# karpathy/minbpe

Hardware: AMD Instinct MI355X
Metric: BPE merges/sec (higher is better)
Workload: dtype int32; 1 GPU; regex1g: RegexTokenizer.train, 1 GB synth seed 2, vocab 32000; mode=default, parallelism=single

## Files before the change

### minbpe_amd/csrc/api/api_basic.hip

```cpp

extern "C" {

const char *bpe_version(void) { return "minbpe_amd libbpe_hip 0.1 (gfx950)"; }

const char *bpe_last_error(bpe_ctx *ctx) { return ctx ? ctx->err.c_str() : g_create_err.c_str(); }

int bpe_create(int device_id, bpe_ctx **out) {
    if (!out) return fail(nullptr, BPE_E_ARG, "out is NULL");
    *out = nullptr;
    int ndev = 0;
    hipError_t e = hipGetDeviceCount(&ndev);
    if (e != hipSuccess || ndev == 0)
        return fail(nullptr, BPE_E_HIP, "no HIP device available: %s",
                    e != hipSuccess ? hipGetErrorString(e) : "device count is 0");
    if (device_id < 0 || device_id >= ndev)
        return fail(nullptr, BPE_E_ARG, "device %d out of range (%d devices)", device_id, ndev);
    bpe_ctx *c = new bpe_ctx();
    c->device = device_id;
    auto bail = [&](const char *what, hipError_t er) {
        int rc = fail(nullptr, BPE_E_HIP, "%s failed: %s", what, hipGetErrorString(er));
        delete c;
        return rc;
    };
    if ((e = hipSetDevice(device_id)) != hipSuccess) return bail("hipSetDevice", e);
    hipDeviceProp_t prop;
    if ((e = hipGetDeviceProperties(&prop, device_id)) != hipSuccess)
        return bail("hipGetDeviceProperties", e);
    c->num_cus = prop.multiProcessorCount > 0 ? prop.multiProcessorCount : 256;
    if (prop.sharedMemPerBlock < (size_t)LEAN_LDS_BYTES) c->lean = 0;
    if ((e = hipStreamCreateWithFlags(&c->stream, hipStreamNonBlocking)) != hipSuccess)
        return bail("hipStreamCreate", e);
    c->own_stream = true;
    for (const void *fn : {(const void *)k_pair_count_lds, (const void *)k_pair_count_bytes, (const void *)k_pair_count_h32})
        if ((e = hipFuncSetAttribute(fn, hipFuncAttributeMaxDynamicSharedMemorySize, PC_LDS_BYTES)) != hipSuccess)
            return bail("hipFuncSetAttribute(dynamic LDS)", e);
    if ((e = hipFuncSetAttribute((const void *)k_load_count, hipFuncAttributeMaxDynamicSharedMemorySize, LC_LDS_BYTES)) != hipSuccess)
        return bail("hipFuncSetAttribute(dynamic LDS)", e);
    if ((e = hipFuncSetAttribute((const void *)bpe::bpe_g4::k_index_build, hipFuncAttributeMaxDynamicSharedMemorySize,
                                 bpe::bpe_g4::IDX_H * 4)) != hipSuccess)
        return bail("hipFuncSetAttribute(dynamic LDS)", e);
    if ((e = hipMalloc((void **)&c->d_st, sizeof(DevState))) != hipSuccess) return bail("hipMalloc", e);
    if ((e = hipMalloc((void **)&c->d_scratch, 8 * sizeof(unsigned long long))) != hipSuccess)
        return bail("hipMalloc", e);
    *out = c;
    return BPE_OK;
}

void bpe_destroy(bpe_ctx *c) {
    if (!c) return;
    (void)hipSetDevice(c->device);
    if (c->stream) (void)hipStreamSynchronize(c->stream);
    if (c->comm) (void)bpe_comm_destroy(c);
    for (ProfEv &ev : c->prof_open) {
        (void)hipEventDestroy(ev.e0);
// ... 448 lines not shown
```

### minbpe_amd/csrc/api/api_train.hip

```cpp

extern "C" {

int bpe_train(bpe_ctx *c, int32_t num_merges, int32_t *pairs_out, uint64_t *counts_out,
              double *iter_ms_out, uint64_t *len_out, int32_t *n_done) {
    if (!c || num_merges < 0) return fail(c, BPE_E_ARG, "bad arguments");
    if (!c->have_bytes) return fail(c, BPE_E_STATE, "bpe_load_bytes first");
    if (c->dp_active) return fail(c, BPE_E_STATE, "bpe_dp_end first");
    static const bool timing = getenv("BPE_TIMING") != nullptr;
    auto now = [] { return std::chrono::steady_clock::now(); };
    auto t_begin = now();
    struct ProfIterReset {
        bpe_ctx *c;
        ~ProfIterReset() { c->prof_iter = -1; }
    } prof_iter_reset{c};
    if (n_done) *n_done = 0;
    HIPCHK(c, hipSetDevice(c->device));
    TRY(ensure_table(c, 256u + (uint32_t)num_merges));
    TRY(ensure_rec(c, std::max(num_merges, 1)));
    memset(c->h_rec, 0, sizeof(IterRec) * (size_t)std::max(num_merges, 1));
    TRY(ensure_srec(c));
    const bool delta = (c->mode == 1);
    EventList ev_list;
    std::vector<hipEvent_t> &evs = ev_list.v;
    struct EvSpan {
// ... 26 lines not shown
    const bool slots = delta && c->use_slots && c->merge_impl == 0;
    const bool form2 = slots && c->use_slots == 2;
    c->idx_live = false;
    c->idx_rebuild = false;
    c->last_count = ~0ull;
    c->n_sparse = c->n_dense = c->n_index_builds = 0;
    c->n_lean = c->n_deferred = 0;
    c->n_steps = c->n_full = c->n_chained = 0;
    c->n_fused = 0;
    static const char *stamp_path = getenv("BPE_STEP_STAMPS");
    const size_t stamp_bytes = (size_t)STEP_STAMP_RING * (3 * 16 + 256 * 2) * sizeof(unsigned long long);
    if (stamp_path) {
        if (!c->d_step_stamps) HIPCHK(c, hipMalloc((void **)&c->d_step_stamps, stamp_bytes));
        HIPCHK(c, hipMemsetAsync(c->d_step_stamps, 0, stamp_bytes, c->stream));
    }
    if (c->d_step_bar) {
        HIPCHK(c, hipMemsetAsync(c->d_step_bar, 0, 256, c->stream));
        c->step_bar_target = 0;
    }
    c->rows_pending = false;
    c->sum_valid = false;
    enum { U_GENERAL = 0, U_LEAN = 1, U_CHAIN = 2 };
    struct Unit {
        int kind;
        int iter;
        uint32_t step;
        uint8_t hdr_flip;
        uint8_t aa_indexed;
        uint8_t pass_kind;
        int ev;
// ... 303 lines not shown
            HIPCHK(c, hipEventElapsedTime(&ms, evs[(size_t)prev], evs[(size_t)sp.ev]));
            for (int j = 0; j < sp.k; j++)
                if (sp.first + j < done) iter_ms_out[sp.first + j] = ms / sp.k;
            prev = sp.ev;
        }
    }
    TRY(prof_drain(c));
    if (stamp_path && c->d_step_stamps) {
        std::vector<unsigned long long> h(stamp_bytes / sizeof(unsigned long long));
        HIPCHK(c, hipMemcpy(h.data(), c->d_step_stamps, stamp_bytes, hipMemcpyDeviceToHost));
        if (FILE *f = fopen(stamp_path, "wb")) {
            fwrite(h.data(), 1, stamp_bytes, f);
            fclose(f);
        }
    }
    if (timing) {
        auto ms = [](auto a, auto b) { return std::chrono::duration<double, std::milli>(b - a).count(); };
        fprintf(stderr, "[bpe_train] %d merges: setup+enqueue of the first pass %.2f ms, loop %.2f ms, drain %.2f ms, "
                        "re-pack + timers %.2f ms\n", done, ms(t_begin, t_loop), ms(t_loop, t_drain), ms(t_drain, t_tail),
                ms(t_tail, now()));
    }
    if (n_done) *n_done = done;
    return rc;
}

}
```

### minbpe_amd/csrc/bpe_device.h

```cpp
#pragma once
#include <stdint.h>

namespace bpe {

constexpr uint32_t FLAG = 0x80000000u;
constexpr uint32_t IDMASK = 0x03FFFFFFu;
constexpr int WSHIFT = 26;
constexpr uint32_t WMASK = 0x7C000000u;
constexpr uint32_t NWMASK = ~WMASK;
constexpr uint32_t INVALID_WORD = 0xFFFFFFFFu;
constexpr uint32_t EMPTY_KEY = 0xFFFFFFFFu;
constexpr unsigned long long NOPOS = ~0ull;

constexpr int MT = 256;
#define BPE_GEOMETRY(NS, MJV, IDXH_LOG2)                                                                         \
    namespace NS {                                                                                               \
    constexpr int MJ = MJV;                            \
    constexpr int WAVE_SPAN = MJ * 256;                                                                          \
    constexpr int TILE = (MT / 64) * WAVE_SPAN;  \
                      \
    constexpr int TILE2 = WAVE_SPAN;                                                                             \
                                  \
    constexpr uint32_t IDX_H = 1u << IDXH_LOG2;                                                                  \
    constexpr int IDX_SHIFT = 32 - IDXH_LOG2;                                                                    \
    }
BPE_GEOMETRY(bpe_g4, 4, 15)
#ifndef BPE_G1_IDXH_LOG2
#define BPE_G1_IDXH_LOG2 13
#endif
BPE_GEOMETRY(bpe_g1, 1, BPE_G1_IDXH_LOG2)
constexpr int TILE2_MAX = 1024, TILE2_MIN = 256;

constexpr int PC_BITS = 14;
constexpr int PC_THREADS = 1024;
constexpr int PC_LDS_BYTES = 131072;
constexpr int PCB_ROUND = 61440;

constexpr int TIE_CAP = 96;
constexpr int ARGMAX_ROWS = 2048;
constexpr uint32_t TIE_WINDOW0 = 0;
constexpr int TIE_BLOCKS = 256;
constexpr int ROW_BLOCKS = 64;
constexpr int DELTA_REPL = 256;
constexpr int DELTA_SKEW = 64;
constexpr int REMOVED_STRIDE = 64;
constexpr int LDSD_CAP = 1920;
// ... 201 lines not shown
```

### minbpe_amd/csrc/kernels/k_chain.hip

```cpp
#include <hip/hip_runtime.h>
#include <stdint.h>

#include "../bpe_device.h"

namespace bpe {
namespace BPE_G {

constexpr uint32_t CH_EX_CAP = 2048;

__device__ __forceinline__ int chain_match(const uint32_t *pa, const uint32_t *pb, uint32_t K, uint32_t w0, uint32_t w1) {
    const uint32_t x = w0 & IDMASK, y = w1 & NWMASK;
    int hit = -1;
    for (uint32_t p = 0; p < K; p++)
        if (x == pa[p] && y == pb[p]) hit = (int)p;
    return (w0 == INVALID_WORD) ? -1 : hit;
}

constexpr uint32_t CH_DCAP = 1024;
constexpr uint32_t CH_SD = 2 * CH_DCAP + 2;
__device__ __forceinline__ void chain_slot_load(const AbArgs &A, const uint32_t t, uint4 (&rv)[MJ], uint4 &hv) {
    const int lane = lane_id();
    const uint32_t *src = A.b0 + (size_t)t * TILE2;
#pragma unroll
    for (int j = 0; j < MJ; j++) rv[j] = *reinterpret_cast<const uint4 *>(src + j * 256 + lane * 4);
    hv = (lane & 1) ? make_uint4(INVALID_WORD, INVALID_WORD, 0u, 0u) : make_uint4(INVALID_WORD, INVALID_WORD, INVALID_WORD, 0u);
    const long long hi = 2ll * (long long)t - 2 + lane;
    if (lane < 6 && hi >= 0 && hi < 2ll * (long long)A.T) hv = reinterpret_cast<const uint4 *>(A.hdr_in)[hi];
}
template <bool DENSE, bool THROUGH = false>
__device__ __forceinline__ void merge_chain_wave(uint32_t *__restrict__ out, uint32_t *__restrict__ sd, const uint32_t t, const AbArgs &A,
                                                 const uint32_t *pa, const uint32_t *pb, const uint32_t *pb1,
                                                 const uint32_t K, const uint32_t z0, const uint32_t brep,
                                                 uint4 (&rv)[MJ], const uint4 hv,
                                                 const uint32_t *ph = nullptr, const uint32_t hm = 0,
                                                 const uint32_t tl_in = 0xFFFFFFFFu) {
    const int lane = lane_id();
    const uint32_t Tl = tl_in != 0xFFFFFFFFu ? tl_in : min(A.T, A.st->tlive);
    const uint32_t *src;
    const uint32_t meta = bcast(hv.w, 2);
    const uint32_t len = meta & 0x7FFFFFFFu, buf = meta >> 31;
    auto keep_header = [&]() {
        if (DENSE && (lane == 2 || lane == 3)) reinterpret_cast<uint4 *>(A.hdr_out)[2 * (size_t)t + (lane - 2)] = hv;
    };
    if (len == 0) {
        keep_header();
        return;
    }
    if (buf) {
        src = A.b1 + (size_t)t * TILE2;
#pragma unroll
        for (int j = 0; j < MJ; j++) rv[j] = *reinterpret_cast<const uint4 *>(src + j * 256 + lane * 4);
    }
    const uint32_t first = bcast(hv.x, 2);
    uint32_t halo0 = bcast(hv.x, 4), halo1 = bcast(hv.y, 4), halo2 = bcast(hv.z, 4);
    uint32_t prev2 = bcast(hv.x, 1), prev1 = bcast(hv.y, 1);
    uint32_t tprev = t - 1;
    uint32_t tnext = t + 1;
    {
        const uint32_t nlen = bcast(hv.w, 4) & 0x7FFFFFFFu, plen = bcast(hv.w, 0) & 0x7FFFFFFFu;
        if ((t + 1 < Tl && nlen < 3) || (t > 0 && plen < 2)) {
            uint32_t ctx[7] = {0, 0, 0, 0, 0, 0, 0};
            if (lane == 0) slot_context_walk(A.hdr_in, t, Tl, ctx);
            halo0 = bcast(ctx[0], 0);
            halo1 = bcast(ctx[1], 0);
            halo2 = bcast(ctx[2], 0);
            prev2 = bcast(ctx[3], 0);
            prev1 = bcast(ctx[4], 0);
            tprev = bcast(ctx[5], 0);
            tnext = bcast(ctx[6], 0);
        }
    }
    auto at = [&](int q, uint32_t own) -> uint32_t {
        const int d = q - (int)len;
        return d < 0 ? own : (d == 0 ? halo0 : (d == 1 ? halo1 : (d == 2 ? halo2 : INVALID_WORD)));
    };
// ... 11 lines not shown
            x[j][1] = at(q0 + 1, rv[j].y);
            x[j][2] = at(q0 + 2, rv[j].z);
            x[j][3] = at(q0 + 3, rv[j].w);
        }
    }
    uint32_t tail[3];
#pragma unroll
    for (int i = 0; i < 3; i++) tail[i] = at(TILE2 + i, 0u);
    uint32_t rb[MJ], jc[MJ], valid[MJ];
#pragma unroll
    for (int j = 0; j < MJ; j++) {
        rb[j] = 0;
        jc[j] = 0;
    }
    uint32_t s = 0;
    uint32_t ia[MJ];
#pragma unroll
    for (int j = 0; j < MJ; j++) ia[j] = 0;
    uint32_t ip = 0;
    if (hm) {
        auto code = [&](uint32_t w) -> uint32_t {
            const uint32_t id = w & IDMASK;
            const uint32_t e = ph[(__umul24(id, hm) >> 8) & 255u];
            return (e >> 8) == id ? (e & 15u) : 0u;
        };
#pragma unroll
        for (int j = 0; j < MJ; j++) {
#pragma unroll
            for (int k = 0; k < 4; k++) ia[j] |= code(x[j][k]) << (4 * k);
        }
        ip = code(prev1);
    } else {
        for (uint32_t p = 0; p < K; p++) {
            const uint32_t a = pa[p];
#pragma unroll
            for (int j = 0; j < MJ; j++) {
#pragma unroll
                for (int k = 0; k < 4; k++) ia[j] |= ((x[j][k] & IDMASK) == a) ? (p + 1u) << (4 * k) : 0u;
            }
            ip = ((prev1 & IDMASK) == a) ? p + 1u : ip;
// ... 14 lines not shown
    }
    s = (uint32_t)((prev1 != INVALID_WORD) & ((first & NWMASK) == pb1[ip]));
#pragma unroll
    for (int j = 0; j < MJ; j++) {
        const int nb = (int)len - (j * 256 + lane * 4);
        valid[j] = nb >= 4 ? 0xFu : (nb <= 0 ? 0u : ((1u << nb) - 1u));
    }
    uint32_t anyr = 0;
#pragma unroll
    for (int j = 0; j < MJ; j++) anyr |= rb[j] & valid[j];
    const bool sites = __any(anyr != 0) != 0;
    if (!sites && !s) {
        keep_header();
        return;
    }
    uint32_t mb[MJ], kb[MJ], ex[MJ], cnt[MJ];
#pragma unroll
    for (int j = 0; j < MJ; j++) {
        mb[j] = rb[j] & valid[j];
        const uint32_t upr = (j > 0) ? ((lane_last(rb[(j + MJ - 1) % MJ]) >> 3) & 1u) : s;
        const uint32_t mp = (uint32_t)dpp_mov<0x138>((int)upr, (int)((rb[j] >> 3) & 1u));
        kb[j] = ~((mb[j] << 1) | mp) & valid[j] & 0xFu;
        cnt[j] = (uint32_t)__popc(kb[j]);
    }
    uint32_t total = 0;
    if constexpr (MJ == 4) {
        const uint32_t i01 = wave_iscan_add(cnt[0] | (cnt[1] << 16));
        const uint32_t i23 = wave_iscan_add(cnt[2] | (cnt[3] << 16));
        const uint32_t t01 = lane_last(i01), t23 = lane_last(i23);
        const uint32_t tot0 = t01 & 0xFFFFu, tot1 = t01 >> 16, tot2 = t23 & 0xFFFFu, tot3 = t23 >> 16;
// ... 165 lines not shown
        __syncthreads();
        if (wave_id() == 0) {
            const uint32_t f = chain_hash_find(s_pa, K);
            if (lane_id() == 0) *s_hm = f;
        }
        __syncthreads();
        hm = *s_hm;
    } else {
        __syncthreads();
    }
    if (hm && threadIdx.x < K) s_ph[(__umul24(s_pa[threadIdx.x], hm) >> 8) & 255u] = (s_pa[threadIdx.x] << 8) | (threadIdx.x + 1u);
    __syncthreads();
    return hm;
}

struct MergeLds {
    alignas(16) uint32_t s_out[LEAN_MT / 64][TILE2];
    uint32_t s_list[LEAN_SUB * 32];
    uint32_t s_tot[2];
    uint32_t s_pa[CH_KMAX], s_pb[CH_KMAX], s_pb1[CH_KMAX + 1];
    uint32_t s_ph[256], s_hm;
};
template <bool THROUGH = false>
__device__ __forceinline__ void merge_chain_body(const AbArgs &A, const uint32_t *__restrict__ idx_dirty, uint32_t use_index,
                                                 MergeLds &L, const uint32_t K, const uint32_t z0, const uint32_t brep,
                                                 const uint32_t blk, const uint32_t nblk, unsigned long long *dbg = nullptr,
                                                 const bool have_st = false, const uint32_t tlive_in = 0, const uint32_t gap_in = 0,
                                                 const bool pre_ok = false, const uint32_t pre_hm = 0) {
    auto dstamp = [&](int i) {
        if (dbg && threadIdx.x == 0) dbg[i] = wall_clock64();
// ... 1 lines not shown
    DevState *st = A.st;
    auto &s_out = L.s_out;
    auto &s_list = L.s_list;
    auto &s_tot = L.s_tot;
    auto &s_pa = L.s_pa;
    auto &s_pb = L.s_pb;
    auto &s_pb1 = L.s_pb1;
    const uint32_t hm = chain_hash_build(L.s_ph, &L.s_hm, s_pa, K, pre_ok, pre_hm);
    const uint32_t *s_ph = L.s_ph;
    const uint32_t Tl = min(A.T, have_st ? tlive_in : st->tlive);
    const uint32_t gap = have_st ? gap_in : st->gap;
    constexpr uint32_t NWV = LEAN_MT / 64;
    AbArgs A1 = A;
    A1.newid = z0;
    const uint32_t a0 = s_pa[0], b0 = s_pb[0];
    auto do_slot = [&](uint32_t t) {
        if (K == 1) {
            merge_ab_wave<true, true, false, THROUGH>(s_out[wave_id()], nullptr, t, A1, a0, b0, Tl);
        } else {
            uint4 rv[MJ], hv;
            chain_slot_load(A, t, rv, hv);
            merge_chain_wave<false, THROUGH>(s_out[wave_id()], nullptr, t, A, s_pa, s_pb, s_pb1, K, z0, brep, rv, hv, s_ph, hm, Tl);
        }
    };
    if (!(use_index & 1u) || gap != 0) {
        const uint32_t nw = nblk * NWV;
        for (uint32_t t = blk * NWV + wave_id(); t < Tl; t += nw) do_slot(t);
        return;
    }
    dstamp(8);
    const uint32_t nwords = (Tl + 31) / 32;
    const uint32_t per = (nwords + nblk - 1) / nblk;
    const uint32_t wlo = blk * per, whi = min(nwords, wlo + per);
    for (uint32_t sub = wlo; sub < whi; sub += LEAN_SUB) {
        uint32_t mk = 0;
        const uint32_t w = sub + threadIdx.x;
        if (threadIdx.x < LEAN_SUB && w < whi) {
            mk = idx_dirty[w];
            for (uint32_t p = 0; p < K; p++) {
                uint32_t h1, h2, h3;
                pair_hash(s_pa[p], s_pb[p], h1, h2, h3);
                mk |= A.idx[(size_t)h1 * A.istride + w] & A.idx[(size_t)h2 * A.istride + w] &
                      A.idx[(size_t)h3 * A.istride + w];
            }
            const uint32_t left = Tl - w * 32;
            if (left < 32) mk &= (1u << left) - 1u;
        }
        const uint32_t c = (uint32_t)__popc(mk);
        const uint32_t inc = wave_iscan_add(c);
        if (threadIdx.x < 128 && lane_id() == 63) s_tot[wave_id()] = inc;
        __syncthreads();
        const uint32_t n = s_tot[0] + s_tot[1];
        if (threadIdx.x < LEAN_SUB) {
            uint32_t o = inc - c + (wave_id() == 1 ? s_tot[0] : 0u);
            while (mk) {
                s_list[o++] = w * 32 + (uint32_t)__ffs((int)mk) - 1u;
                mk &= mk - 1u;
            }
        }
        __syncthreads();
        if (sub == wlo) dstamp(9);
        if (K == 1 || MJ > 1 || !(use_index & 2u)) {
            for (uint32_t i = wave_id(); i < n; i += NWV) do_slot(s_list[i]);
        } else {
            uint32_t i = wave_id();
            uint4 rv[MJ], hv, nrv[MJ], nhv;
            if (i < n) chain_slot_load(A, s_list[i], rv, hv);
            for (; i < n; i += NWV) {
                const bool more = i + NWV < n;
                if (more) chain_slot_load(A, s_list[i + NWV], nrv, nhv);
                merge_chain_wave<false, THROUGH>(s_out[wave_id()], nullptr, s_list[i], A, s_pa, s_pb, s_pb1, K, z0, brep, rv, hv, s_ph, hm, Tl);
                if (more) {
#pragma unroll
                    for (int j = 0; j < MJ; j++) rv[j] = nrv[j];
                    hv = nhv;
                }
            }
        }
        __syncthreads();
    }
}
enum { SW_BK = 48, SW_BZ0, SW_BREP, SW_STATUS, SW_DEFER, SW_SEL_RAN, SW_TLIVE, SW_GAP, SW_BHM, SW_BHM_KEY, SW_ADJ, SW_N };
static_assert(SW_N <= 64, "one wave fetches the state words");
__device__ __forceinline__ void step_words_fetch(const DevState *st, uint32_t *s_w) {
    const uint32_t i = threadIdx.x;
    if (i < (uint32_t)SW_N) {
        const uint32_t *base = reinterpret_cast<const uint32_t *>(st);
        uint32_t off;
        if (i < 16) off = (uint32_t)offsetof(DevState, ba) / 4 + i;
        else if (i < 32) off = (uint32_t)offsetof(DevState, bb) / 4 + (i - 16);
        else if (i < 48) off = (uint32_t)offsetof(DevState, badj) / 4 + (i - 32);
        else {
            constexpr uint32_t o[SW_N - 48] = {
                (uint32_t)offsetof(DevState, bk) / 4,      (uint32_t)offsetof(DevState, bz0) / 4,     (uint32_t)offsetof(DevState, brep) / 4,
                (uint32_t)offsetof(DevState, status) / 4,  (uint32_t)offsetof(DevState, defer) / 4,   (uint32_t)offsetof(DevState, sel_ran) / 4,
// ... 545 lines not shown
```

### minbpe_amd/csrc/kernels/k_index.hip

```cpp
#include <hip/hip_runtime.h>
#include <stdint.h>

#include "../bpe_device.h"

namespace bpe {
namespace BPE_G {

static_assert((1u << (32 - IDX_SHIFT)) == IDX_H, "hash width");
__device__ __forceinline__ void pair_hash(uint32_t x, uint32_t y, uint32_t &h1, uint32_t &h2, uint32_t &h3) {
    h1 = ((x * 0x9E3779B1u) ^ (y * 0x85EBCA77u)) >> IDX_SHIFT;
    h2 = ((x * 0xC2B2AE3Du) + (y * 0x27D4EB2Fu) + 0x165667B1u) >> IDX_SHIFT;
    h3 = (((x + 0x7F4A7C15u) * 0xD6E8FEB9u) ^ ((y + 0x51ED270Bu) * 0xA24BAED5u)) >> IDX_SHIFT;
}
__device__ __forceinline__ void index_add(uint32_t *__restrict__ idx, uint32_t stride, uint32_t owner, uint32_t x,
                                          uint32_t y) {
    uint32_t h1, h2, h3;
    pair_hash(x, y, h1, h2, h3);
    const uint32_t g = owner >> 5, bit = 1u << (owner & 31);
    atomicOr(&idx[(size_t)h1 * stride + g], bit);
    atomicOr(&idx[(size_t)h2 * stride + g], bit);
    atomicOr(&idx[(size_t)h3 * stride + g], bit);
#ifdef BPE_DUMMY_ATOMICS
    atomicOr(&idx[(size_t)(h1 ^ 1u) * stride + g], 0u);
    atomicOr(&idx[(size_t)(h2 ^ 1u) * stride + g], 0u);
    atomicOr(&idx[(size_t)(h3 ^ 1u) * stride + g], 0u);
#endif
}

__device__ __forceinline__ void build_cand_list(const CandArgs &C, DevState *st, uint32_t a, uint32_t b) {
    __shared__ uint32_t s_wtot[16];
    __shared__ uint32_t s_base;
    const uint32_t nwords = (C.T + 31) / 32;
    uint32_t h1, h2, h3;
    pair_hash(a, b, h1, h2, h3);
    const bool all = st->gap != 0;
    if (threadIdx.x == 0) s_base = 0;
    __syncthreads();
    constexpr int GP = 4;
    for (uint32_t base = 0; base < nwords; base += GP * 1024) {
        uint32_t m[GP] = {0, 0, 0, 0};
        uint32_t c = 0;
        const uint32_t w4 = base + GP * threadIdx.x;
        uint32_t mnext = 0;
        if (a == b && w4 + GP < nwords && !all)
            mnext = (C.idx[(size_t)h1 * C.stride + w4 + GP] & C.idx[(size_t)h2 * C.stride + w4 + GP] &
                     C.idx[(size_t)h3 * C.stride + w4 + GP]) | C.dirty[w4 + GP];
        if (w4 < nwords && !all) {
            const uint4 r1 = *reinterpret_cast<const uint4 *>(C.idx + (size_t)h1 * C.stride + w4);
            const uint4 r2 = *reinterpret_cast<const uint4 *>(C.idx + (size_t)h2 * C.stride + w4);
            const uint4 r3 = *reinterpret_cast<const uint4 *>(C.idx + (size_t)h3 * C.stride + w4);
            const uint4 d = *reinterpret_cast<const uint4 *>(C.dirty + w4);
            m[0] = (r1.x & r2.x & r3.x) | d.x;
            m[1] = (r1.y & r2.y & r3.y) | d.y;
            m[2] = (r1.z & r2.z & r3.z) | d.z;
            m[3] = (r1.w & r2.w & r3.w) | d.w;
            if (a == b) {
                m[0] |= (m[0] >> 1) | (m[1] << 31);
                m[1] |= (m[1] >> 1) | (m[2] << 31);
                m[2] |= (m[2] >> 1) | (m[3] << 31);
                m[3] |= (m[3] >> 1) | (mnext << 31);
            }
        }
#pragma unroll
        for (int u = 0; u < GP; u++) {
            const uint32_t w = w4 + u;
            if (w < nwords) {
                if (all) m[u] = 0xFFFFFFFFu;
                const uint32_t left = C.T - w * 32;
                if (left < 32) m[u] &= (1u << left) - 1u;
            } else {
// ... 32 lines not shown
```

### minbpe_amd/csrc/kernels/k_lean.hip

```cpp
#include <hip/hip_runtime.h>
#include <stdint.h>

#include "../bpe_device.h"

namespace bpe {
namespace BPE_G {

constexpr uint32_t NOROW = 0xFFFFFFFFu;
constexpr int DBITS_WORDS = 2048;
constexpr uint32_t LEAN_EX_CAP = 1024;
constexpr uint32_t LEAN_SUM_CAP = 1024;
constexpr uint32_t LEAN_CHAIN_TIES = 48;
constexpr uint32_t LEAN_BLK_CAP = 128;

constexpr int LEAN_MT = 1024;
constexpr uint32_t LEAN_SUB = 128;
constexpr int LEAN_LDS_BYTES = (LEAN_MT / 64) * TILE2 * 4 + (int)LEAN_SUB * 32 * 4 + 8;
static_assert(LEAN_LDS_BYTES <= 160 * 1024, "k_merge_ab_lean: staging + candidate list must fit the CU's LDS");
template <bool INDEXED>
__global__ void __launch_bounds__(LEAN_MT)
k_merge_ab_lean(AbArgs A, const uint32_t *__restrict__ idx_dirty, uint32_t use_index, uint32_t *__restrict__ dbits) {
    __shared__ __attribute__((aligned(16))) uint32_t s_out[LEAN_MT / 64][TILE2];
    __shared__ uint32_t s_list[LEAN_SUB * 32];
    __shared__ uint32_t s_tot[2];
// ... 13 lines not shown
    if (a == b) {
        if (blockIdx.x == 0 && threadIdx.x == 0) st->defer = 1;
        return;
    }
    const uint32_t Tl = min(A.T, st->tlive);
    constexpr uint32_t NWV = LEAN_MT / 64;
    if (!use_index || st->gap != 0) {
        const uint32_t nw = gridDim.x * NWV;
        for (uint32_t t = blockIdx.x * NWV + wave_id(); t < Tl; t += nw)
            merge_ab_wave<true, INDEXED, false>(s_out[wave_id()], nullptr, t, A, a, b, Tl);
        return;
    }
    const uint32_t nwords = (Tl + 31) / 32;
    const uint32_t per = (nwords + gridDim.x - 1) / gridDim.x;
    const uint32_t wlo = blockIdx.x * per, whi = min(nwords, wlo + per);
    uint32_t h1, h2, h3;
    pair_hash(a, b, h1, h2, h3);
    for (uint32_t sub = wlo; sub < whi; sub += LEAN_SUB) {
        uint32_t mk = 0;
        const uint32_t w = sub + threadIdx.x;
        if (threadIdx.x < LEAN_SUB && w < whi) {
            mk = (A.idx[(size_t)h1 * A.istride + w] & A.idx[(size_t)h2 * A.istride + w] &
                  A.idx[(size_t)h3 * A.istride + w]) | idx_dirty[w];
            const uint32_t left = Tl - w * 32;
            if (left < 32) mk &= (1u << left) - 1u;
        }
        const uint32_t c = (uint32_t)__popc(mk);
        const uint32_t inc = wave_iscan_add(c);
        if (threadIdx.x < 128 && lane_id() == 63) s_tot[wave_id()] = inc;
        __syncthreads();
        const uint32_t n = s_tot[0] + s_tot[1];
        if (threadIdx.x < LEAN_SUB) {
            uint32_t o = inc - c + (wave_id() == 1 ? s_tot[0] : 0u);
            while (mk) {
                s_list[o++] = w * 32 + (uint32_t)__ffs((int)mk) - 1u;
                mk &= mk - 1u;
            }
        }
// ... 648 lines not shown
```

### minbpe_amd/csrc/kernels/k_select.hip

```cpp
#include <hip/hip_runtime.h>
#include <stdint.h>

#include "../bpe_device.h"

namespace bpe {
namespace BPE_G {


__device__ __forceinline__ bool slot_get(const SlotRef &r, uint64_t n, uint64_t p, uint32_t &w) {
    if (!r.meta) {
        if (p >= n) return false;
        w = r.b0[p];
        return true;
    }
    const uint64_t t = p / TILE;
    if (t >= r.T) return false;
    const uint32_t m = r.meta[t];
    if ((uint32_t)(p % TILE) >= (m & 0x7FFFFFFFu)) return false;
    w = ((m >> 31) ? r.b1 : r.b0)[p];
    return true;
}
__device__ __forceinline__ bool slot_next(const SlotRef &r, uint64_t n, uint64_t p, uint32_t &w) {
    if (!r.meta) return slot_get(r, n, p + 1, w);
    uint64_t t = p / TILE;
// ... 239 lines not shown
    }
    return NOPOS;
}

__device__ __forceinline__ unsigned long long tie_by_index(const SlotRefH &ref, const CandArgs &C,
                                                          const int32_t *s_tied, uint32_t nt,
                                                          unsigned long long *s_pos = nullptr) {
    __shared__ unsigned long long s_best;
    if (threadIdx.x == 0) s_best = NOPOS;
    __syncthreads();
    const int lane = lane_id();
    const uint32_t nwords = (C.T + 31) / 32;
    const bool all = s_pos != nullptr;
    for (uint32_t p = wave_id(); p < nt; p += 16) {
        const uint32_t x = (uint32_t)s_tied[2 * p], y = (uint32_t)s_tied[2 * p + 1];
        uint32_t h1, h2, h3;
        pair_hash(x, y, h1, h2, h3);
        unsigned long long found = NOPOS;
        bool done = false;
        for (uint32_t wb = 0; wb < nwords && !done; wb += 64) {
            if (!all && (__atomic_load_n(&s_best, __ATOMIC_RELAXED) >> 7) < (unsigned long long)wb * 32 * TILE2) break;
            const uint32_t w = wb + lane;
            uint32_t mk = 0;
            if (w < nwords) {
                mk = (C.idx[(size_t)h1 * C.stride + w] & C.idx[(size_t)h2 * C.stride + w] &
                      C.idx[(size_t)h3 * C.stride + w]) | C.dirty[w];
                const uint32_t left = C.T - w * 32;
                if (left < 32) mk &= (1u << left) - 1u;
            }
            unsigned long long bal = __ballot(mk != 0);
            while (bal && !done) {
                const int lw = __ffsll((long long)bal) - 1;
                bal &= bal - 1;
                uint32_t mm = (uint32_t)__builtin_amdgcn_readlane((int)mk, lw);
                while (mm) {
                    const uint32_t t = (wb + lw) * 32 + (uint32_t)__ffs((int)mm) - 1u;
                    mm &= mm - 1u;
                    if (!all && (__atomic_load_n(&s_best, __ATOMIC_RELAXED) >> 7) < (unsigned long long)t * TILE2) {
                        done = true;
                        break;
                    }
// ... 290 lines not shown
```

### minbpe_amd/csrc/kernels/k_slots2.hip

```cpp
#include <hip/hip_runtime.h>
#include <stdint.h>

#include "../bpe_device.h"

namespace bpe {
namespace BPE_G {



__global__ void __launch_bounds__(256)
k_slot2_init(SlotHdr *__restrict__ hdr, uint64_t T, DevState *st, int par, uint32_t which,
             const uint32_t *__restrict__ ids) {
    const uint64_t n = st->n[par];
    if (blockIdx.x == 0 && threadIdx.x == 0) {
        st->gap = 0;
        st->tlive = (uint32_t)min(T, (n + TILE2 - 1) / TILE2);
    }
    const uint64_t stride = (uint64_t)gridDim.x * blockDim.x;
    for (uint64_t t = (uint64_t)blockIdx.x * blockDim.x + threadIdx.x; t < T; t += stride) {
        const uint64_t b0 = t * TILE2;
        const uint32_t len = b0 >= n ? 0u : (uint32_t)min((uint64_t)TILE2, n - b0);
        SlotHdr h;
        h.w0 = len > 0 ? ids[b0] : INVALID_WORD;
        h.w1 = len > 1 ? ids[b0 + 1] : INVALID_WORD;
// ... 49 lines not shown
    ctx[1] = h1;
    ctx[2] = h2;
    ctx[3] = p2;
    ctx[4] = p1;
    ctx[5] = tp;
    ctx[6] = tn;
}

__device__ __forceinline__ uint32_t bcast(uint32_t v, int srclane) {
    return (uint32_t)__builtin_amdgcn_readlane((int)v, srclane);
}

template <bool SPARSE, bool INDEXED, bool LDSD, bool THROUGH = false>
__device__ __forceinline__ void merge_ab_wave(uint32_t *__restrict__ out, uint32_t *__restrict__ sd, const uint32_t t,
                                              const AbArgs &A, const uint32_t a, const uint32_t b,
                                              const uint32_t tl_in = 0xFFFFFFFFu) {
    const int lane = lane_id();
    const uint32_t Tl = tl_in != 0xFFFFFFFFu ? tl_in : min(A.T, A.st->tlive);
    const uint32_t *src = A.b0 + (size_t)t * TILE2;
    uint4 rv[MJ];
#pragma unroll
    for (int j = 0; j < MJ; j++) rv[j] = *reinterpret_cast<const uint4 *>(src + j * 256 + lane * 4);
    uint4 hv = (lane & 1) ? make_uint4(INVALID_WORD, INVALID_WORD, 0u, 0u)
                          : make_uint4(INVALID_WORD, INVALID_WORD, INVALID_WORD, 0u);
    {
        const long long hi = 2ll * (long long)t - 2 + lane;
        if (lane < 6 && hi >= 0 && hi < 2ll * (long long)A.T) hv = reinterpret_cast<const uint4 *>(A.hdr_in)[hi];
    }
    const uint32_t meta = bcast(hv.w, 2);
    const uint32_t len = meta & 0x7FFFFFFFu, buf = meta >> 31;
    auto keep_header = [&]() {
// ... 61 lines not shown
        for (int k = 0; k < 4; k++) {
            const uint32_t nxt = (k < 3) ? x[j][k + 1] : nx;
            r |= (uint32_t)(((x[j][k] & IDMASK) == a) & ((nxt & NWMASK) == b)) << k;
        }
        const int nb = (int)len - (j * 256 + lane * 4);
        valid[j] = nb >= 4 ? 0xFu : (nb <= 0 ? 0u : ((1u << nb) - 1u));
        rb[j] = r;
        anyr |= r & valid[j];
    }
    const uint32_t s = (uint32_t)((prev1 != INVALID_WORD) & ((prev1 & IDMASK) == a) & ((first & NWMASK) == b));
    const bool sites = __any(anyr != 0) != 0;
    if (!sites && !s) {
        keep_header();
        return;
    }
    uint32_t mb[MJ], kb[MJ], ex[MJ], cnt[MJ];
#pragma unroll
    for (int j = 0; j < MJ; j++) {
        mb[j] = rb[j] & valid[j];
        const uint32_t upr = (j > 0) ? ((lane_last(rb[(j + MJ - 1) % MJ]) >> 3) & 1u) : s;
        const uint32_t mp = (uint32_t)dpp_mov<0x138>((int)upr, (int)((rb[j] >> 3) & 1u));
        kb[j] = ~((mb[j] << 1) | mp) & valid[j] & 0xFu;
        cnt[j] = (uint32_t)__popc(kb[j]);
    }
    uint32_t total = 0;
    if constexpr (MJ == 4) {
        const uint32_t i01 = wave_iscan_add(cnt[0] | (cnt[1] << 16));
        const uint32_t i23 = wave_iscan_add(cnt[2] | (cnt[3] << 16));
        const uint32_t t01 = lane_last(i01), t23 = lane_last(i23);
        const uint32_t tot0 = t01 & 0xFFFFu, tot1 = t01 >> 16, tot2 = t23 & 0xFFFFu, tot3 = t23 >> 16;
// ... 478 lines not shown
            }
            const uint32_t d = len - q;
#pragma unroll
            for (int k = 1; k <= 4; k++)
                if ((uint32_t)k == d) x[k] = nxt;
        }
        const uint32_t bit = 1u << sl;
        if (q == 0 && t > 0 && !(x[0] & FLAG)) {
            uint32_t pw = INVALID_WORD;
            for (uint32_t u = t; u-- > 0;) {
                if (hdr[u].meta & 0x7FFFFFFFu) {
                    pw = hdr[u].l1;
                    break;
                }
            }
            if (pw != INVALID_WORD) {
                uint32_t h1, h2, h3;
                pair_hash(pw & IDMASK, x[0] & IDMASK, h1, h2, h3);
                atomicOr(&s_mask[h1], bit);
                atomicOr(&s_mask[h2], bit);
                atomicOr(&s_mask[h3], bit);
            }
        }
#pragma unroll
        for (int k = 0; k < 4; k++) {
            if (q + k < len && !(x[k + 1] & FLAG)) {
                uint32_t h1, h2, h3;
                pair_hash(x[k] & IDMASK, x[k + 1] & IDMASK, h1, h2, h3);
                atomicOr(&s_mask[h1], bit);
                atomicOr(&s_mask[h2], bit);
                atomicOr(&s_mask[h3], bit);
            }
        }
    }
    __syncthreads();
    uint32_t *row = scratch + (size_t)g * IDX_H;
    for (uint32_t i = threadIdx.x; i < IDX_H; i += 1024) row[i] = s_mask[i];
}

__global__ void __launch_bounds__(256)
k_index_transpose(const uint32_t *__restrict__ scratch, uint32_t ngroups, uint32_t *__restrict__ idx,
                  uint32_t stride) {
    __shared__ uint32_t tile[32][33];
    const uint32_t g0 = blockIdx.x * 32, h0 = blockIdx.y * 32;
    const uint32_t tx = threadIdx.x & 31, ty = threadIdx.x >> 5;
#pragma unroll
    for (int i = 0; i < 4; i++) {
// ... 33 lines not shown
```

Measured before the change: 51940 merges/s.

## Add early-reject in chain merge and retune g1 Bloom index geometry

Adds an early-reject path in merge_chain_wave that, when no context walk is needed, checks whether any token in the slot matches a chain left-id and returns before loading halos and running the full merge. It also changes the g1 Bloom index to twice as many rows with two hash functions instead of three, which cuts row reads and atomics per lookup and insert. The hash helpers are made generic over the hash count, and opt-in visit-stat counters are added behind a compile flag. The risks are a higher false-positive rate from fewer hashes, a larger index memory footprint, and extra halo-patch logic on the early path.

Result: slower. 50650 merges/s (-2.5%).

```diff
diff --git a/minbpe_amd/csrc/api/api_basic.hip b/minbpe_amd/csrc/api/api_basic.hip
--- a/minbpe_amd/csrc/api/api_basic.hip
+++ b/minbpe_amd/csrc/api/api_basic.hip
@@ -38,6 +38,9 @@
         return bail("hipFuncSetAttribute(dynamic LDS)", e);
     if ((e = hipFuncSetAttribute((const void *)bpe::bpe_g4::k_index_build, hipFuncAttributeMaxDynamicSharedMemorySize,
                                  bpe::bpe_g4::IDX_H * 4)) != hipSuccess)
+        return bail("hipFuncSetAttribute(dynamic LDS)", e);
+    if ((e = hipFuncSetAttribute((const void *)bpe::bpe_g1::k_index_build, hipFuncAttributeMaxDynamicSharedMemorySize,
+                                 bpe::bpe_g1::IDX_H * 4)) != hipSuccess)
         return bail("hipFuncSetAttribute(dynamic LDS)", e);
     if ((e = hipMalloc((void **)&c->d_st, sizeof(DevState))) != hipSuccess) return bail("hipMalloc", e);
     if ((e = hipMalloc((void **)&c->d_scratch, 8 * sizeof(unsigned long long))) != hipSuccess)
diff --git a/minbpe_amd/csrc/api/api_train.hip b/minbpe_amd/csrc/api/api_train.hip
--- a/minbpe_amd/csrc/api/api_train.hip
+++ b/minbpe_amd/csrc/api/api_train.hip
@@ -64,6 +64,14 @@
         if (!c->d_step_stamps) HIPCHK(c, hipMalloc((void **)&c->d_step_stamps, stamp_bytes));
         HIPCHK(c, hipMemsetAsync(c->d_step_stamps, 0, stamp_bytes, c->stream));
     }
+#ifdef BPE_VISIT_STATS
+    static const char *visit_path = getenv("BPE_VISIT_STATS");
+    {
+        const unsigned long long z[VS_PHASES * VS_COUNTERS] = {};
+        HIPCHK(c, hipMemcpyToSymbol(HIP_SYMBOL(bpe::bpe_g1::g_visit_stats), z, sizeof(z)));
+        HIPCHK(c, hipMemcpyToSymbol(HIP_SYMBOL(bpe::bpe_g4::g_visit_stats), z, sizeof(z)));
+    }
+#endif
     if (c->d_step_bar) {
         HIPCHK(c, hipMemsetAsync(c->d_step_bar, 0, 256, c->stream));
         c->step_bar_target = 0;
@@ -397,6 +405,30 @@
             fclose(f);
         }
     }
+#ifdef BPE_VISIT_STATS
+    if (visit_path) {
+        unsigned long long v[2][VS_PHASES * VS_COUNTERS];
+        HIPCHK(c, hipMemcpyFromSymbol(v[0], HIP_SYMBOL(bpe::bpe_g1::g_visit_stats), sizeof(v[0])));
+        HIPCHK(c, hipMemcpyFromSymbol(v[1], HIP_SYMBOL(bpe::bpe_g4::g_visit_stats), sizeof(v[1])));
+        if (FILE *f = fopen(visit_path, "w")) {
+            static const char *const names[VS_COUNTERS] = {"visited", "live", "dirty_only", "filter_empty", "dirty_only_live", "passes"};
+            static const char *const phases[VS_PHASES] = {"0-300", "300-1000", "1000-4000", "4000-16000", "16000-end"};
+            fprintf(f, "{\"merges\": %d", done);
+            for (int g = 0; g < 2; g++) {
+                fprintf(f, ", \"%s\": {", g ? "g4" : "g1");
+                for (int p = 0; p < VS_PHASES; p++) {
+                    fprintf(f, "%s\"%s\": {", p ? ", " : "", phases[p]);
+                    for (int i = 0; i < VS_COUNTERS; i++)
+                        fprintf(f, "%s\"%s\": %llu", i ? ", " : "", names[i], v[g][p * VS_COUNTERS + i]);
+                    fprintf(f, "}");
+                }
+                fprintf(f, "}");
+            }
+            fprintf(f, "}\n");
+            fclose(f);
+        }
+    }
+#endif
     if (timing) {
         auto ms = [](auto a, auto b) { return std::chrono::duration<double, std::milli>(b - a).count(); };
         fprintf(stderr, "[bpe_train] %d merges: setup+enqueue of the first pass %.2f ms, loop %.2f ms, drain %.2f ms, "
diff --git a/minbpe_amd/csrc/bpe_device.h b/minbpe_amd/csrc/bpe_device.h
--- a/minbpe_amd/csrc/bpe_device.h
+++ b/minbpe_amd/csrc/bpe_device.h
@@ -13,23 +13,33 @@
 constexpr unsigned long long NOPOS = ~0ull;
 
 constexpr int MT = 256;
-#define BPE_GEOMETRY(NS, MJV, IDXH_LOG2)                                                                         \
+#define BPE_GEOMETRY(NS, MJV, IDXH_LOG2, IDXK)                                                                   \
     namespace NS {                                                                                               \
     constexpr int MJ = MJV;                            \
     constexpr int WAVE_SPAN = MJ * 256;                                                                          \
     constexpr int TILE = (MT / 64) * WAVE_SPAN;  \
                       \
     constexpr int TILE2 = WAVE_SPAN;                                                                             \
-                                  \
+        \
     constexpr uint32_t IDX_H = 1u << IDXH_LOG2;                                                                  \
     constexpr int IDX_SHIFT = 32 - IDXH_LOG2;                                                                    \
+    constexpr int IDX_K = IDXK;                                                                                  \
+    static_assert(IDX_K == 2 || IDX_K == 3, "pair_hash (k_index.hip) has three hash functions");                \
     }
-BPE_GEOMETRY(bpe_g4, 4, 15)
+BPE_GEOMETRY(bpe_g4, 4, 15, 3)
 #ifndef BPE_G1_IDXH_LOG2
-#define BPE_G1_IDXH_LOG2 13
+#define BPE_G1_IDXH_LOG2 14
 #endif
-BPE_GEOMETRY(bpe_g1, 1, BPE_G1_IDXH_LOG2)
+#ifndef BPE_G1_IDX_K
+#define BPE_G1_IDX_K 2
+#endif
+BPE_GEOMETRY(bpe_g1, 1, BPE_G1_IDXH_LOG2, BPE_G1_IDX_K)
 constexpr int TILE2_MAX = 1024, TILE2_MIN = 256;
+#ifndef BPE_EARLY_REJECT
+#define BPE_EARLY_REJECT 1
+#endif
+constexpr int VS_PHASES = 5, VS_COUNTERS = 6;
+enum { VS_VISITED = 0, VS_LIVE, VS_DIRTY_ONLY, VS_FILTER_EMPTY, VS_DIRTY_ONLY_LIVE, VS_PASSES };
 
 constexpr int PC_BITS = 14;
 constexpr int PC_THREADS = 1024;
diff --git a/minbpe_amd/csrc/kernels/k_chain.hip b/minbpe_amd/csrc/kernels/k_chain.hip
--- a/minbpe_amd/csrc/kernels/k_chain.hip
+++ b/minbpe_amd/csrc/kernels/k_chain.hip
@@ -33,7 +33,7 @@
                                                  const uint32_t K, const uint32_t z0, const uint32_t brep,
                                                  uint4 (&rv)[MJ], const uint4 hv,
                                                  const uint32_t *ph = nullptr, const uint32_t hm = 0,
-                                                 const uint32_t tl_in = 0xFFFFFFFFu) {
+                                                 const uint32_t tl_in = 0xFFFFFFFFu, uint32_t *hit = nullptr) {
     const int lane = lane_id();
     const uint32_t Tl = tl_in != 0xFFFFFFFFu ? tl_in : min(A.T, A.st->tlive);
     const uint32_t *src;
@@ -52,13 +52,59 @@
         for (int j = 0; j < MJ; j++) rv[j] = *reinterpret_cast<const uint4 *>(src + j * 256 + lane * 4);
     }
     const uint32_t first = bcast(hv.x, 2);
+    uint32_t prev1 = bcast(hv.y, 1);
+    const uint32_t nlen = bcast(hv.w, 4) & 0x7FFFFFFFu, plen = bcast(hv.w, 0) & 0x7FFFFFFFu;
+    const bool walk = (t + 1 < Tl && nlen < 3) || (t > 0 && plen < 2);
+    auto code = [&](uint32_t w) -> uint32_t {
+        const uint32_t id = w & IDMASK;
+        const uint32_t e = ph[(__umul24(id, hm) >> 8) & 255u];
+        return (e >> 8) == id ? (e & 15u) : 0u;
+    };
+    uint32_t ia[MJ];
+#pragma unroll
+    for (int j = 0; j < MJ; j++) ia[j] = 0;
+    uint32_t ip = 0;
+    bool early = false;
+    if constexpr (!DENSE && BPE_EARLY_REJECT) early = !walk;
+    if (early) {
+        uint32_t vn[MJ];
+#pragma unroll
+        for (int j = 0; j < MJ; j++) {
+            const int nb = (int)len - (j * 256 + lane * 4);
+            vn[j] = nb >= 4 ? 0xFFFFu : (nb <= 0 ? 0u : ((1u << (4 * nb)) - 1u));
+        }
+        if (hm) {
+#pragma unroll
+            for (int j = 0; j < MJ; j++) ia[j] = code(rv[j].x) | (code(rv[j].y) << 4) | (code(rv[j].z) << 8) | (code(rv[j].w) << 12);
+            ip = code(prev1);
+        } else {
+            for (uint32_t p = 0; p < K; p++) {
+                const uint32_t a = pa[p];
+#pragma unroll
+                for (int j = 0; j < MJ; j++) {
+                    ia[j] |= ((rv[j].x & IDMASK) == a) ? (p + 1u) : 0u;
+                    ia[j] |= ((rv[j].y & IDMASK) == a) ? (p + 1u) << 4 : 0u;
+                    ia[j] |= ((rv[j].z & IDMASK) == a) ? (p + 1u) << 8 : 0u;
+                    ia[j] |= ((rv[j].w & IDMASK) == a) ? (p + 1u) << 12 : 0u;
+                }
+                ip = ((prev1 & IDMASK) == a) ? p + 1u : ip;
+            }
+        }
+        uint32_t anyf = 0;
+#pragma unroll
+        for (int j = 0; j < MJ; j++) {
+            ia[j] &= vn[j];
+            anyf |= ia[j];
+        }
+        const uint32_t s_e = (uint32_t)((prev1 != INVALID_WORD) & ((first & NWMASK) == pb1[ip]));
+        if (!__any(anyf != 0) && !s_e) return;
+    }
     uint32_t halo0 = bcast(hv.x, 4), halo1 = bcast(hv.y, 4), halo2 = bcast(hv.z, 4);
-    uint32_t prev2 = bcast(hv.x, 1), prev1 = bcast(hv.y, 1);
+    uint32_t prev2 = bcast(hv.x, 1);
     uint32_t tprev = t - 1;
     uint32_t tnext = t + 1;
     {
-        const uint32_t nlen = bcast(hv.w, 4) & 0x7FFFFFFFu, plen = bcast(hv.w, 0) & 0x7FFFFFFFu;
-        if ((t + 1 < Tl && nlen < 3) || (t > 0 && plen < 2)) {
+        if (walk) {
             uint32_t ctx[7] = {0, 0, 0, 0, 0, 0, 0};
             if (lane == 0) slot_context_walk(A.hdr_in, t, Tl, ctx);
             halo0 = bcast(ctx[0], 0);
@@ -100,16 +146,23 @@
         jc[j] = 0;
     }
     uint32_t s = 0;
-    uint32_t ia[MJ];
-#pragma unroll
-    for (int j = 0; j < MJ; j++) ia[j] = 0;
-    uint32_t ip = 0;
-    if (hm) {
-        auto code = [&](uint32_t w) -> uint32_t {
-            const uint32_t id = w & IDMASK;
-            const uint32_t e = ph[(__umul24(id, hm) >> 8) & 255u];
-            return (e >> 8) == id ? (e & 15u) : 0u;
-        };
+    if (early) {
+        uint32_t hc = 0;
+        const uint32_t hw = lane == 0 ? halo0 : (lane == 1 ? halo1 : halo2);
+        if (hm) {
+            hc = code(hw);
+        } else {
+            for (uint32_t p = 0; p < K; p++) hc = ((hw & IDMASK) == pa[p]) ? p + 1u : hc;
+        }
+        const uint32_t hcode = bcast(hc, 0) | (bcast(hc, 1) << 4) | (bcast(hc, 2) << 8);
+#pragma unroll
+        for (int j = 0; j < MJ; j++) {
+            if ((j + 1) * 256 <= (int)len) continue;
+            const int sh = 4 * ((int)len - (j * 256 + lane * 4));
+            const uint32_t patch = sh >= 16 || sh <= -12 ? 0u : (sh >= 0 ? hcode << sh : hcode >> (-sh));
+            ia[j] |= patch & 0xFFFFu;
+        }
+    } else if (hm) {
 #pragma unroll
         for (int j = 0; j < MJ; j++) {
 #pragma unroll
@@ -154,6 +207,7 @@
         keep_header();
         return;
     }
+    if (hit) *hit = 1;
     uint32_t mb[MJ], kb[MJ], ex[MJ], cnt[MJ];
 #pragma unroll
     for (int j = 0; j < MJ; j++) {
@@ -349,6 +403,9 @@
     return hm;
 }
 
+#ifdef BPE_VISIT_STATS
+__device__ unsigned long long g_visit_stats[VS_PHASES * VS_COUNTERS];
+#endif
 struct MergeLds {
     alignas(16) uint32_t s_out[LEAN_MT / 64][TILE2];
     uint32_t s_list[LEAN_SUB * 32];
@@ -380,18 +437,54 @@
     AbArgs A1 = A;
     A1.newid = z0;
     const uint32_t a0 = s_pa[0], b0 = s_pb[0];
-    auto do_slot = [&](uint32_t t) {
+#ifdef BPE_VISIT_STATS
+    uint32_t vs[VS_COUNTERS] = {0, 0, 0, 0, 0, 0};
+    auto vs_note = [&](uint32_t e, uint32_t live, bool listed) {
+        vs[VS_VISITED]++;
+        vs[VS_LIVE] += live;
+        if (listed) {
+            vs[VS_DIRTY_ONLY] += e >> 31;
+            vs[VS_DIRTY_ONLY_LIVE] += (e >> 31) & live;
+            vs[VS_FILTER_EMPTY] += (~e >> 31) & (live ^ 1u);
+        }
+    };
+    auto vs_flush = [&]() {
+        const uint32_t m = z0 - 256u;
+        const uint32_t ph = m < 300 ? 0 : (m < 1000 ? 1 : (m < 4000 ? 2 : (m < 16000 ? 3 : 4)));
+        if (lane_id() == 0) {
+            for (int i = 0; i < VS_PASSES; i++)
+                if (vs[i]) atomicAdd(&g_visit_stats[ph * VS_COUNTERS + i], (unsigned long long)vs[i]);
+            if (blk == 0 && threadIdx.x == 0) atomicAdd(&g_visit_stats[ph * VS_COUNTERS + VS_PASSES], 1ull);
+        }
+    };
+#define VS_SLOT(e) ((e) & 0x7FFFFFFFu)
+#define VS_HIT_ARG , &vs_hit
+#else
+#define VS_SLOT(e) (e)
+#define VS_HIT_ARG
+#endif
+    auto do_slot = [&](uint32_t e, bool listed) {
+        const uint32_t t = VS_SLOT(e);
+#ifdef BPE_VISIT_STATS
+        uint32_t vs_hit = 0;
+#endif
         if (K == 1) {
-            merge_ab_wave<true, true, false, THROUGH>(s_out[wave_id()], nullptr, t, A1, a0, b0, Tl);
+            merge_ab_wave<true, true, false, THROUGH>(s_out[wave_id()], nullptr, t, A1, a0, b0, Tl VS_HIT_ARG);
         } else {
             uint4 rv[MJ], hv;
             chain_slot_load(A, t, rv, hv);
-            merge_chain_wave<false, THROUGH>(s_out[wave_id()], nullptr, t, A, s_pa, s_pb, s_pb1, K, z0, brep, rv, hv, s_ph, hm, Tl);
-        }
+            merge_chain_wave<false, THROUGH>(s_out[wave_id()], nullptr, t, A, s_pa, s_pb, s_pb1, K, z0, brep, rv, hv, s_ph, hm, Tl VS_HIT_ARG);
+        }
+#ifdef BPE_VISIT_STATS
+        vs_note(e, vs_hit, listed);
+#endif
     };
     if (!(use_index & 1u) || gap != 0) {
         const uint32_t nw = nblk * NWV;
-        for (uint32_t t = blk * NWV + wave_id(); t < Tl; t += nw) do_slot(t);
+        for (uint32_t t = blk * NWV + wave_id(); t < Tl; t += nw) do_slot(t, false);
+#ifdef BPE_VISIT_STATS
+        vs_flush();
+#endif
         return;
     }
     dstamp(8);
@@ -401,14 +494,19 @@
     for (uint32_t sub = wlo; sub < whi; sub += LEAN_SUB) {
         uint32_t mk = 0;
         const uint32_t w = sub + threadIdx.x;
+#ifdef BPE_VISIT_STATS
+        uint32_t mk_filter = 0;
+#endif
         if (threadIdx.x < LEAN_SUB && w < whi) {
-            mk = idx_dirty[w];
             for (uint32_t p = 0; p < K; p++) {
-                uint32_t h1, h2, h3;
-                pair_hash(s_pa[p], s_pb[p], h1, h2, h3);
-                mk |= A.idx[(size_t)h1 * A.istride + w] & A.idx[(size_t)h2 * A.istride + w] &
-                      A.idx[(size_t)h3 * A.istride + w];
-            }
+                uint32_t h[IDX_K];
+                pair_hash(s_pa[p], s_pb[p], h);
+                mk |= index_rows(A.idx, A.istride, h, w);
+            }
+#ifdef BPE_VISIT_STATS
+            mk_filter = mk;
+#endif
+            mk |= idx_dirty[w];
             const uint32_t left = Tl - w * 32;
             if (left < 32) mk &= (1u << left) - 1u;
         }
@@ -420,22 +518,33 @@
         if (threadIdx.x < LEAN_SUB) {
             uint32_t o = inc - c + (wave_id() == 1 ? s_tot[0] : 0u);
             while (mk) {
-                s_list[o++] = w * 32 + (uint32_t)__ffs((int)mk) - 1u;
+                const uint32_t sb = (uint32_t)__ffs((int)mk) - 1u;
+#ifdef BPE_VISIT_STATS
+                s_list[o++] = (w * 32 + sb) | (((~mk_filter >> sb) & 1u) << 31);
+#else
+                s_list[o++] = w * 32 + sb;
+#endif
                 mk &= mk - 1u;
             }
         }
         __syncthreads();
         if (sub == wlo) dstamp(9);
         if (K == 1 || MJ > 1 || !(use_index & 2u)) {
-            for (uint32_t i = wave_id(); i < n; i += NWV) do_slot(s_list[i]);
+            for (uint32_t i = wave_id(); i < n; i += NWV) do_slot(s_list[i], true);
         } else {
             uint32_t i = wave_id();
             uint4 rv[MJ], hv, nrv[MJ], nhv;
-            if (i < n) chain_slot_load(A, s_list[i], rv, hv);
+            if (i < n) chain_slot_load(A, VS_SLOT(s_list[i]), rv, hv);
             for (; i < n; i += NWV) {
                 const bool more = i + NWV < n;
-                if (more) chain_slot_load(A, s_list[i + NWV], nrv, nhv);
-                merge_chain_wave<false, THROUGH>(s_out[wave_id()], nullptr, s_list[i], A, s_pa, s_pb, s_pb1, K, z0, brep, rv, hv, s_ph, hm, Tl);
+                if (more) chain_slot_load(A, VS_SLOT(s_list[i + NWV]), nrv, nhv);
+#ifdef BPE_VISIT_STATS
+                uint32_t vs_hit = 0;
+#endif
+                merge_chain_wave<false, THROUGH>(s_out[wave_id()], nullptr, VS_SLOT(s_list[i]), A, s_pa, s_pb, s_pb1, K, z0, brep, rv, hv, s_ph, hm, Tl VS_HIT_ARG);
+#ifdef BPE_VISIT_STATS
+                vs_note(s_list[i], vs_hit, true);
+#endif
                 if (more) {
 #pragma unroll
                     for (int j = 0; j < MJ; j++) rv[j] = nrv[j];
@@ -445,6 +554,11 @@
         }
         __syncthreads();
     }
+#ifdef BPE_VISIT_STATS
+    vs_flush();
+#endif
+#undef VS_SLOT
+#undef VS_HIT_ARG
 }
 enum { SW_BK = 48, SW_BZ0, SW_BREP, SW_STATUS, SW_DEFER, SW_SEL_RAN, SW_TLIVE, SW_GAP, SW_BHM, SW_BHM_KEY, SW_ADJ, SW_N };
 static_assert(SW_N <= 64, "one wave fetches the state words");
diff --git a/minbpe_amd/csrc/kernels/k_index.hip b/minbpe_amd/csrc/kernels/k_index.hip
--- a/minbpe_amd/csrc/kernels/k_index.hip
+++ b/minbpe_amd/csrc/kernels/k_index.hip
@@ -7,32 +7,56 @@
 namespace BPE_G {
 
 static_assert((1u << (32 - IDX_SHIFT)) == IDX_H, "hash width");
-__device__ __forceinline__ void pair_hash(uint32_t x, uint32_t y, uint32_t &h1, uint32_t &h2, uint32_t &h3) {
-    h1 = ((x * 0x9E3779B1u) ^ (y * 0x85EBCA77u)) >> IDX_SHIFT;
-    h2 = ((x * 0xC2B2AE3Du) + (y * 0x27D4EB2Fu) + 0x165667B1u) >> IDX_SHIFT;
-    h3 = (((x + 0x7F4A7C15u) * 0xD6E8FEB9u) ^ ((y + 0x51ED270Bu) * 0xA24BAED5u)) >> IDX_SHIFT;
+__device__ __forceinline__ void pair_hash(uint32_t x, uint32_t y, uint32_t (&h)[IDX_K]) {
+    h[0] = ((x * 0x9E3779B1u) ^ (y * 0x85EBCA77u)) >> IDX_SHIFT;
+    h[1] = ((x * 0xC2B2AE3Du) + (y * 0x27D4EB2Fu) + 0x165667B1u) >> IDX_SHIFT;
+    if constexpr (IDX_K > 2) h[2] = (((x + 0x7F4A7C15u) * 0xD6E8FEB9u) ^ ((y + 0x51ED270Bu) * 0xA24BAED5u)) >> IDX_SHIFT;
 }
 __device__ __forceinline__ void index_add(uint32_t *__restrict__ idx, uint32_t stride, uint32_t owner, uint32_t x,
                                           uint32_t y) {
-    uint32_t h1, h2, h3;
-    pair_hash(x, y, h1, h2, h3);
+    uint32_t h[IDX_K];
+    pair_hash(x, y, h);
     const uint32_t g = owner >> 5, bit = 1u << (owner & 31);
-    atomicOr(&idx[(size_t)h1 * stride + g], bit);
-    atomicOr(&idx[(size_t)h2 * stride + g], bit);
-    atomicOr(&idx[(size_t)h3 * stride + g], bit);
+#pragma unroll
+    for (int k = 0; k < IDX_K; k++) atomicOr(&idx[(size_t)h[k] * stride + g], bit);
 #ifdef BPE_DUMMY_ATOMICS
-    atomicOr(&idx[(size_t)(h1 ^ 1u) * stride + g], 0u);
-    atomicOr(&idx[(size_t)(h2 ^ 1u) * stride + g], 0u);
-    atomicOr(&idx[(size_t)(h3 ^ 1u) * stride + g], 0u);
+#pragma unroll
+    for (int k = 0; k < IDX_K; k++) atomicOr(&idx[(size_t)(h[k] ^ 1u) * stride + g], 0u);
 #endif
+}
+__device__ __forceinline__ void index_fill(uint32_t *s_mask, uint32_t bit, uint32_t x, uint32_t y) {
+    uint32_t h[IDX_K];
+    pair_hash(x, y, h);
+#pragma unroll
+    for (int k = 0; k < IDX_K; k++) atomicOr(&s_mask[h[k]], bit);
+}
+__device__ __forceinline__ uint32_t index_rows(const uint32_t *__restrict__ idx, uint32_t stride, const uint32_t (&h)[IDX_K],
+                                               uint32_t w) {
+    uint32_t m = idx[(size_t)h[0] * stride + w];
+#pragma unroll
+    for (int k = 1; k < IDX_K; k++) m &= idx[(size_t)h[k] * stride + w];
+    return m;
+}
+__device__ __forceinline__ uint4 index_rows4(const uint32_t *__restrict__ idx, uint32_t stride, const uint32_t (&h)[IDX_K],
+                                             uint32_t w) {
+    uint4 m = *reinterpret_cast<const uint4 *>(idx + (size_t)h[0] * stride + w);
+#pragma unroll
+    for (int k = 1; k < IDX_K; k++) {
+        const uint4 r = *reinterpret_cast<const uint4 *>(idx + (size_t)h[k] * stride + w);
+        m.x &= r.x;
+        m.y &= r.y;
+        m.z &= r.z;
+        m.w &= r.w;
+    }
+    return m;
 }
 
 __device__ __forceinline__ void build_cand_list(const CandArgs &C, DevState *st, uint32_t a, uint32_t b) {
     __shared__ uint32_t s_wtot[16];
     __shared__ uint32_t s_base;
     const uint32_t nwords = (C.T + 31) / 32;
-    uint32_t h1, h2, h3;
-    pair_hash(a, b, h1, h2, h3);
+    uint32_t h[IDX_K];
+    pair_hash(a, b, h);
     const bool all = st->gap != 0;
     if (threadIdx.x == 0) s_base = 0;
     __syncthreads();
@@ -43,17 +67,14 @@
         const uint32_t w4 = base + GP * threadIdx.x;
         uint32_t mnext = 0;
         if (a == b && w4 + GP < nwords && !all)
-            mnext = (C.idx[(size_t)h1 * C.stride + w4 + GP] & C.idx[(size_t)h2 * C.stride + w4 + GP] &
-                     C.idx[(size_t)h3 * C.stride + w4 + GP]) | C.dirty[w4 + GP];
+            mnext = index_rows(C.idx, C.stride, h, w4 + GP) | C.dirty[w4 + GP];
         if (w4 < nwords && !all) {
-            const uint4 r1 = *reinterpret_cast<const uint4 *>(C.idx + (size_t)h1 * C.stride + w4);
-            const uint4 r2 = *reinterpret_cast<const uint4 *>(C.idx + (size_t)h2 * C.stride + w4);
-            const uint4 r3 = *reinterpret_cast<const uint4 *>(C.idx + (size_t)h3 * C.stride + w4);
+            const uint4 r = index_rows4(C.idx, C.stride, h, w4);
             const uint4 d = *reinterpret_cast<const uint4 *>(C.dirty + w4);
-            m[0] = (r1.x & r2.x & r3.x) | d.x;
-            m[1] = (r1.y & r2.y & r3.y) | d.y;
-            m[2] = (r1.z & r2.z & r3.z) | d.z;
-            m[3] = (r1.w & r2.w & r3.w) | d.w;
+            m[0] = r.x | d.x;
+            m[1] = r.y | d.y;
+            m[2] = r.z | d.z;
+            m[3] = r.w | d.w;
             if (a == b) {
                 m[0] |= (m[0] >> 1) | (m[1] << 31);
                 m[1] |= (m[1] >> 1) | (m[2] << 31);
diff --git a/minbpe_amd/csrc/kernels/k_lean.hip b/minbpe_amd/csrc/kernels/k_lean.hip
--- a/minbpe_amd/csrc/kernels/k_lean.hip
+++ b/minbpe_amd/csrc/kernels/k_lean.hip
@@ -51,14 +51,13 @@
     const uint32_t nwords = (Tl + 31) / 32;
     const uint32_t per = (nwords + gridDim.x - 1) / gridDim.x;
     const uint32_t wlo = blockIdx.x * per, whi = min(nwords, wlo + per);
-    uint32_t h1, h2, h3;
-    pair_hash(a, b, h1, h2, h3);
+    uint32_t h[IDX_K];
+    pair_hash(a, b, h);
     for (uint32_t sub = wlo; sub < whi; sub += LEAN_SUB) {
         uint32_t mk = 0;
         const uint32_t w = sub + threadIdx.x;
         if (threadIdx.x < LEAN_SUB && w < whi) {
-            mk = (A.idx[(size_t)h1 * A.istride + w] & A.idx[(size_t)h2 * A.istride + w] &
-                  A.idx[(size_t)h3 * A.istride + w]) | idx_dirty[w];
+            mk = index_rows(A.idx, A.istride, h, w) | idx_dirty[w];
             const uint32_t left = Tl - w * 32;
             if (left < 32) mk &= (1u << left) - 1u;
         }
diff --git a/minbpe_amd/csrc/kernels/k_select.hip b/minbpe_amd/csrc/kernels/k_select.hip
--- a/minbpe_amd/csrc/kernels/k_select.hip
+++ b/minbpe_amd/csrc/kernels/k_select.hip
@@ -277,8 +277,8 @@
     const bool all = s_pos != nullptr;
     for (uint32_t p = wave_id(); p < nt; p += 16) {
         const uint32_t x = (uint32_t)s_tied[2 * p], y = (uint32_t)s_tied[2 * p + 1];
-        uint32_t h1, h2, h3;
-        pair_hash(x, y, h1, h2, h3);
+        uint32_t h[IDX_K];
+        pair_hash(x, y, h);
         unsigned long long found = NOPOS;
         bool done = false;
         for (uint32_t wb = 0; wb < nwords && !done; wb += 64) {
@@ -286,8 +286,7 @@
             const uint32_t w = wb + lane;
             uint32_t mk = 0;
             if (w < nwords) {
-                mk = (C.idx[(size_t)h1 * C.stride + w] & C.idx[(size_t)h2 * C.stride + w] &
-                      C.idx[(size_t)h3 * C.stride + w]) | C.dirty[w];
+                mk = index_rows(C.idx, C.stride, h, w) | C.dirty[w];
                 const uint32_t left = C.T - w * 32;
                 if (left < 32) mk &= (1u << left) - 1u;
             }
diff --git a/minbpe_amd/csrc/kernels/k_slots2.hip b/minbpe_amd/csrc/kernels/k_slots2.hip
--- a/minbpe_amd/csrc/kernels/k_slots2.hip
+++ b/minbpe_amd/csrc/kernels/k_slots2.hip
@@ -87,7 +87,7 @@
 template <bool SPARSE, bool INDEXED, bool LDSD, bool THROUGH = false>
 __device__ __forceinline__ void merge_ab_wave(uint32_t *__restrict__ out, uint32_t *__restrict__ sd, const uint32_t t,
                                               const AbArgs &A, const uint32_t a, const uint32_t b,
-                                              const uint32_t tl_in = 0xFFFFFFFFu) {
+                                              const uint32_t tl_in = 0xFFFFFFFFu, uint32_t *hit = nullptr) {
     const int lane = lane_id();
     const uint32_t Tl = tl_in != 0xFFFFFFFFu ? tl_in : min(A.T, A.st->tlive);
     const uint32_t *src = A.b0 + (size_t)t * TILE2;
@@ -179,6 +179,7 @@
         keep_header();
         return;
     }
+    if (hit) *hit = 1;
     uint32_t mb[MJ], kb[MJ], ex[MJ], cnt[MJ];
 #pragma unroll
     for (int j = 0; j < MJ; j++) {
@@ -687,23 +688,11 @@
                     break;
                 }
             }
-            if (pw != INVALID_WORD) {
-                uint32_t h1, h2, h3;
-                pair_hash(pw & IDMASK, x[0] & IDMASK, h1, h2, h3);
-                atomicOr(&s_mask[h1], bit);
-                atomicOr(&s_mask[h2], bit);
-                atomicOr(&s_mask[h3], bit);
-            }
+            if (pw != INVALID_WORD) index_fill(s_mask, bit, pw & IDMASK, x[0] & IDMASK);
         }
 #pragma unroll
         for (int k = 0; k < 4; k++) {
-            if (q + k < len && !(x[k + 1] & FLAG)) {
-                uint32_t h1, h2, h3;
-                pair_hash(x[k] & IDMASK, x[k + 1] & IDMASK, h1, h2, h3);
-                atomicOr(&s_mask[h1], bit);
-                atomicOr(&s_mask[h2], bit);
-                atomicOr(&s_mask[h3], bit);
-            }
+            if (q + k < len && !(x[k + 1] & FLAG)) index_fill(s_mask, bit, x[k] & IDMASK, x[k + 1] & IDMASK);
         }
     }
     __syncthreads();
```
